# TritonDataCenter/containerpilot

Measured on AMD Instinct MI355X. Metric: events/sec, higher is better.
Workload: dtype n/a (CPU daemon, no tensor math; see BASELINE.json north_star); 1 GPU; model=containerpilot daemon, BASELINE stress shape scaled to 550 jobs, jobs=550, watches=50, parallelism=1 independent daemons (1/rank)

## Files before the change

### cpp/include/cpilot/jobs.hpp

```cpp
#pragma once

#include <functional>
#include <memory>
#include <string>
#include <vector>

#include "cpilot/command.hpp"
#include "cpilot/discovery.hpp"
#include "cpilot/events.hpp"
#include "cpilot/json.hpp"
#include "cpilot/probe.hpp"
#include "cpilot/timing.hpp"

namespace cpilot {

constexpr int kUnlimited = -1;

enum class JobStatus {
  Idle = 0,
  Unknown,
  Healthy,
  Unhealthy,
  Maintenance,
  AlwaysHealthy,
  Completed,
};
const char* jobStatusString(JobStatus s);

struct JobConfig {
  std::string name;
  CommandPtr exec;

  int port = 0;
  std::string initialStatus;
  std::vector<std::string> tags;
  std::shared_ptr<ServiceDefinition> serviceDefinition;

  CommandPtr healthCheckExec;
  health::ProbePtr healthProbe;
// ... 101 lines not shown
```

### cpp/include/cpilot/loop.hpp

```cpp
#pragma once

#include <sys/types.h>

#include <chrono>
#include <cstdint>
#include <deque>
#include <functional>
#include <map>
#include <memory>
#include <mutex>
#include <queue>
#include <vector>

namespace cpilot {

using Clock = std::chrono::steady_clock;
using TimePoint = Clock::time_point;
using Ns = std::chrono::nanoseconds;

std::function<void()> timedItem(const char* tag, std::function<void()> fn);
void dumpItemTags();

void resetThreadScheduling();

class Loop {
 public:
  using FdCallback = std::function<void(uint32_t epollEvents)>;
  using TimerCallback = std::function<void()>;
  using ChildCallback = std::function<void(int waitStatus)>;

  Loop();
  ~Loop();

  Loop(const Loop&) = delete;
  Loop& operator=(const Loop&) = delete;

  void watchFd(int fd, uint32_t events, FdCallback cb);
  void modifyFd(int fd, uint32_t events);
  void unwatchFd(int fd);

  uint64_t addTimeout(Ns delay, TimerCallback cb);
  uint64_t addInterval(Ns interval, TimerCallback cb, Ns initialDelay = Ns(-1));
  void cancelTimer(uint64_t id);

  void defer(std::function<void()> fn);

  void post(std::function<void()> fn);

  void watchChild(pid_t pid, ChildCallback cb);
  void reapChildren();
  void notifyChildExit(pid_t pid, int status);

  static void postIfLive(Loop* loop, uint64_t id, std::function<void()> fn);
  uint64_t id() const { return id_; }

  void run();
  void stop();

  bool stopped() const { return stopped_; }

 private:
  struct Timer {
    uint64_t id;
    TimePoint deadline;
    Ns interval;
    TimerCallback cb;
    bool canceled = false;
  };
  struct TimerCmp {
    bool operator()(const std::shared_ptr<Timer>& a,
                    const std::shared_ptr<Timer>& b) const {
      return a->deadline > b->deadline;
    }
  };

  void armTimerFd();
  void fireDueTimers();
  void drainDeferred();
  void drainPosted();

  uint64_t id_ = 0;
  int epfd_ = -1;
  int timerfd_ = -1;
  int wakeupFds_[2] = {-1, -1};
  bool stopped_ = false;

  std::map<int, FdCallback> fdCallbacks_;
  std::priority_queue<std::shared_ptr<Timer>,
                      std::vector<std::shared_ptr<Timer>>, TimerCmp>
      timers_;
  std::map<uint64_t, std::shared_ptr<Timer>> timersById_;
  uint64_t nextTimerId_ = 1;

  std::deque<std::function<void()>> deferred_;

  std::mutex postedMu_;
  std::deque<std::function<void()>> posted_;

  std::map<pid_t, ChildCallback> children_;
  std::map<pid_t, int> unclaimedExits_;
};

}
```

### cpp/include/cpilot/spawner.hpp

```cpp
#pragma once

#include <sys/types.h>

#include <cstdint>
#include <deque>
#include <functional>
#include <map>
#include <memory>
#include <mutex>
#include <string>
#include <thread>
#include <vector>

#include "cpilot/loop.hpp"

namespace cpilot {

class Spawner {
 public:
  using SpawnCb = std::function<void(pid_t pid, int err)>;

  static Spawner& global();

  void spawn(Loop& loop, const std::string& execPath,
             const std::vector<std::string>& args,
             std::shared_ptr<const std::vector<std::string>> baseEnv,
// ... 4 lines not shown

  size_t backlog();
  bool overloaded();

 private:
  Spawner();
  struct Helper {
    int sock = -1;
    pid_t pid = -1;
    bool dead = false;
    std::deque<std::pair<std::vector<char>, int>> overflow;
    std::mutex sendMu;
  };
  struct Pending {
    Loop* loop;
    uint64_t loopId;
    SpawnCb cb;
    size_t helperIdx;
  };

  bool launchHelper(Helper* h);
  void flushOverflow(size_t idx);
  void readerMain();
  void handleMessage(size_t idx, const char* buf, size_t len);
  void helperDied(size_t idx);
  bool sendRequest(Helper& h, const std::vector<char>& buf, int fd);
  void wakeReader();

  std::string helperPath_;
  std::vector<std::unique_ptr<Helper>> helpers_;
  size_t nextHelper_ = 0;

  std::mutex mu_;
  std::map<uint32_t, Pending> pending_;
  uint32_t nextReqId_ = 1;
  std::map<pid_t, std::pair<Loop*, uint64_t>> pidLoops_;

  int wakeFds_[2] = {-1, -1};
  std::thread reader_;
};

}
```

### cpp/src/discovery.cpp

```cpp
#include "cpilot/discovery.hpp"

#include <algorithm>
#include <cstdlib>
#include <thread>

#include "cpilot/decode.hpp"
#include "cpilot/http.hpp"
#include "cpilot/log.hpp"

namespace cpilot {

namespace {

void parseRawURI(const std::string& raw, std::string* address,
                 std::string* scheme) {
  *scheme = "http";
  *address = raw;
  if (raw.rfind("http://", 0) == 0) {
    *address = raw.substr(7);
  } else if (raw.rfind("https://", 0) == 0) {
    *address = raw.substr(8);
    *scheme = "https";
  }
}
// ... 134 lines not shown
    blockingReg_ = std::make_shared<BlockingReg>();
  for (int i = 0; i < 4; i++)
    workers_.emplace_back([this] { workerMain(); });
}

void ConsulBackend::stop() {
  {
    std::lock_guard<std::mutex> l(mu_);
    if (stopping_ && workers_.empty()) return;
    stopping_ = true;
  }
  {
    std::lock_guard<std::mutex> l(blockingReg_->mu);
    blockingReg_->stopping = true;
    for (auto& t : blockingReg_->tokens) t->cancel();
  }
  cv_.notify_all();
  for (auto& t : workers_) t.join();
  workers_.clear();
}

void ConsulBackend::workerMain() {
  resetThreadScheduling();
  while (true) {
    std::function<void()> task;
    {
      std::unique_lock<std::mutex> l(mu_);
      cv_.wait(l, [this] { return stopping_ || !tasks_.empty(); });
      if (stopping_ && tasks_.empty()) return;
      auto& front = tasks_.front();
      if (!front.first.empty()) queuedKeys_.erase(front.first);
      task = std::move(front.second);
      tasks_.pop_front();
    }
    task();
  }
}

bool ConsulBackend::enqueue(const std::string& key,
                            std::function<void()> task) {
  {
    std::lock_guard<std::mutex> l(mu_);
    if (stopping_) return false;
    if (!key.empty() && !queuedKeys_.insert(key).second) return false;
    if (tasks_.size() >= 10000) {
      if (++dropped_ % 1000 == 1)
// ... 173 lines not shown
                                          HealthBlockingCb cb) {
  std::string path = "/v1/health/service/" + urlEncode(name) + "?passing=1";
  if (!tag.empty()) path += "&tag=" + urlEncode(tag);
  if (!dc.empty()) path += "&dc=" + urlEncode(dc);
  path += "&index=" + std::to_string(lastIndex) +
          "&wait=" + std::to_string(waitSeconds) + "s";
  auto token = std::make_shared<http::CancelToken>();
  auto reg = blockingReg_;
  {
    std::lock_guard<std::mutex> l(reg->mu);
    if (reg->stopping) {
      loop_->post([cb] { cb(false, {}, 0); });
      return;
    }
    reg->tokens.insert(token);
  }
  std::string target = address_;
  std::string tokenHdr = token_;
  http::TlsOptions tls = tls_;
  Loop* loop = loop_;
  std::thread([reg, target, tokenHdr, tls, path, cb, loop, token,
               waitSeconds] {
    resetThreadScheduling();
    std::map<std::string, std::string> headers;
    if (!tokenHdr.empty()) headers["X-Consul-Token"] = tokenHdr;
    auto res = http::request(target, "GET", path, "", "application/json",
                             headers, (waitSeconds + 10) * 1000, &tls,
                             token.get());
    {
      std::lock_guard<std::mutex> l(reg->mu);
      reg->tokens.erase(token);
    }
    bool ok = res.ok && res.status == 200 && !token->cancelled();
    uint64_t index = 0;
    auto it = res.headers.find("x-consul-index");
    if (it != res.headers.end())
      index = strtoull(it->second.c_str(), nullptr, 10);
    std::vector<ServiceEntry> entries;
    if (ok) entries = parseHealthEntries(res.body, &ok);
    loop->post([cb, ok, index, entries = std::move(entries)]() mutable {
      cb(ok, std::move(entries), index);
    });
  }).detach();
}

bool ConsulBackend::compareAndSwap(const std::string& service,
// ... 68 lines not shown
```

### cpp/src/events.cpp

```cpp
#include "cpilot/events.hpp"

#include <algorithm>
#include <cstdio>

#include "cpilot/log.hpp"

namespace cpilot {

const Event GlobalStartup{EventCode::Startup, "global"};
const Event GlobalShutdown{EventCode::Shutdown, "global"};
const Event NonEvent{EventCode::None, ""};
const Event GlobalEnterMaintenance{EventCode::EnterMaintenance, "global"};
const Event GlobalExitMaintenance{EventCode::ExitMaintenance, "global"};
const Event QuitByTest{EventCode::Quit, "closed"};

const char* eventCodeString(EventCode code) {
  switch (code) {
    case EventCode::None: return "None";
    case EventCode::ExitSuccess: return "ExitSuccess";
    case EventCode::ExitFailed: return "ExitFailed";
    case EventCode::Stopping: return "Stopping";
    case EventCode::Stopped: return "Stopped";
    case EventCode::StatusHealthy: return "StatusHealthy";
    case EventCode::StatusUnhealthy: return "StatusUnhealthy";
// ... 66 lines not shown
        tombstones_ = true;
      }
    }
  };
  tombstone(wildcard_);
  for (auto& kv : bySource_) tombstone(kv.second);
  for (auto& kv : byCode_) tombstone(kv.second);
}

void Bus::publish(Event event) {
  LOG_DEBUG("event: %s", event.str().c_str());
  if (event.code != EventCode::Metric) {
    eventsCounter_->inc({eventCodeString(event.code), event.source});
  }
  published_++;
  ring_[(head_ + 1) % (int)ring_.size()] = event;
  int old = head_;
  head_ = (head_ + 1) % (int)ring_.size();
  if (old != -1 && head_ == tail_) tail_ = (tail_ + 1) % (int)ring_.size();

  queue_.emplace_back(std::move(event), Clock::now());
  if (!drainScheduled_) {
    drainScheduled_ = true;
    loop_.defer([self = shared_from_this()] { self->drain(); });
  }
}

void Bus::drain() {
  drainScheduled_ = false;
  constexpr auto kBudget = std::chrono::milliseconds(2);
  TimePoint start = Clock::now();
  size_t n = queue_.size();
  for (size_t i = 0; i < n && !queue_.empty(); i++) {
    if ((i & 63) == 63 && Clock::now() - start >= kBudget) break;
    auto [event, publishedAt] = std::move(queue_.front());
    queue_.pop_front();
    double latency =
        std::chrono::duration<double>(Clock::now() - publishedAt).count();
    dispatchHist_->observe(latency);
    static const bool latDebug = cpilotDebugEnv("CPILOT_LOOP_DEBUG");
    if (latDebug && latency > 0.004)
      fprintf(stderr, "slow dispatch: %s waited %.1f ms (queue %zu)\n",
              event.str().c_str(), latency * 1e3, queue_.size());
    latencySeen_++;
    if (latencyWindow_.size() < latencyCap_) {
      latencyWindow_.push_back(latency);
    } else {
      uint64_t slot = latencyRng_() % latencySeen_;
      if (slot < latencyCap_) latencyWindow_[slot] = latency;
    }
    size_t srcHash = std::hash<std::string>{}(event.source);
    uint64_t seq = ++seq_;
    uint64_t batch = 0;
    deliverList(wildcard_, event, srcHash, seq, &batch);
    auto codeIt = byCode_.find((int)event.code);
    if (codeIt != byCode_.end())
      deliverList(codeIt->second, event, srcHash, seq, &batch);
    auto srcIt = bySource_.find(srcHash);
    if (srcIt != bySource_.end())
      deliverList(srcIt->second, event, srcHash, seq, &batch);
    if (batch) deliveriesCounter_->inc({}, (double)batch);
  }
  if (tombstones_) compactIndexes();
  if (!queue_.empty() && !drainScheduled_) {
    drainScheduled_ = true;
    loop_.defer([self = shared_from_this()] { self->drain(); });
  }
}

void Bus::deliverList(std::vector<Subscriber*>& list, const Event& event,
                      size_t srcHash, uint64_t seq, uint64_t* batch) {
  size_t bound = list.size();
  for (size_t si = 0; si < bound; si++) {
    Subscriber* s = list[si];
    if (!s || s->busSeq_ == seq) continue;
    s->busSeq_ = seq;
    delivered_++;
    (*batch)++;
    s->onEventHashed(event, srcHash);
  }
}

void Bus::compactIndexes() {
  auto compact = [](std::vector<Subscriber*>& list) {
    list.erase(std::remove(list.begin(), list.end(), nullptr), list.end());
  };
  compact(wildcard_);
  for (auto it = bySource_.begin(); it != bySource_.end();) {
    compact(it->second);
    it = it->second.empty() ? bySource_.erase(it) : std::next(it);
// ... 27 lines not shown
```

### cpp/src/jobs.cpp

```cpp
#include "cpilot/jobs.hpp"

#include <unistd.h>

#include <cstring>

#include "cpilot/decode.hpp"
#include "cpilot/ips.hpp"
#include "cpilot/log.hpp"
#include "cpilot/spawner.hpp"

namespace cpilot {

const char* jobStatusString(JobStatus s) {
  switch (s) {
    case JobStatus::Healthy: return "healthy";
    case JobStatus::Unhealthy: return "unhealthy";
    case JobStatus::Maintenance: return "maintenance";
    case JobStatus::AlwaysHealthy: return "healthy";
    case JobStatus::Completed: return "completed";
    default: return "unknown";
  }
}


// ... 505 lines not shown
      startTimeout_(cfg->whenTimeout),
      startsRemain_(cfg->whenStartsLimit),
      stoppingWaitEvent_(cfg->stoppingWaitEvent),
      stoppingTimeout_(cfg->stoppingTimeout),
      heartbeat_(cfg->heartbeatInterval),
      restartLimit_(cfg->restartLimit),
      restartsRemain_(cfg->restartLimit),
      frequency_(cfg->freqInterval) {
  heartbeatSource_ = name_ + ".heartbeat";
  runEverySource_ = name_ + ".run-every";
  healthCheckName_ =
      healthCheckExec_ ? healthCheckExec_->name() : ("check." + name_);
  stoppingTimeoutSource_ = name_ + ".stopping-timeout";
  std::hash<std::string> h;
  hName_ = h(name_);
  hHeartbeat_ = h(heartbeatSource_);
  hRunEvery_ = h(runEverySource_);
  hCheck_ = h(healthCheckName_);
  if (name_ == "containerpilot") {
    status_ = JobStatus::AlwaysHealthy;
  }
}

Subscription Job::subscription() const {
  Subscription sub;
  sub.all = false;
  sub.sources = {name_,          healthCheckName_,
                 heartbeatSource_, runEverySource_,
                 stoppingTimeoutSource_, name_ + ".wait-timeout"};
  if (!startEvent_.source.empty()) sub.sources.push_back(startEvent_.source);
  if (stoppingWaitEvent_ != NonEvent)
    sub.sources.push_back(stoppingWaitEvent_.source);
  sub.codes = {EventCode::Quit, EventCode::Shutdown,
               EventCode::EnterMaintenance, EventCode::ExitMaintenance,
               EventCode::Signal};
  return sub;
}

void Job::run(Loop& loop, std::shared_ptr<Bus> bus,
              std::function<void()> completedCb) {
  loop_ = &loop;
  bus_ = std::move(bus);
  completedCb_ = std::move(completedCb);
  auto self = shared_from_this();

  auto phase = [this](Duration interval) {
    uint64_t h = std::hash<std::string>{}(name_);
    return Duration(interval.count() / 2 +
                    (Ns::rep)(h % 1000) * interval.count() / 2000);
  };

  if (frequency_ > Duration(0)) {
    freqTimer_ = loop.addInterval(frequency_, [this, self] {
      LOG_DEBUG("timer: {TimerExpired %s.run-every}", name_.c_str());
      processEvent(Event{EventCode::TimerExpired, runEverySource_});
    }, phase(frequency_));
  }
  if (heartbeat_ > Duration(0)) {
    heartbeatTimer_ = loop.addInterval(heartbeat_, [this, self] {
      if (name_ != "containerpilot")
        LOG_DEBUG("timer: {TimerExpired %s.heartbeat}", name_.c_str());
      processEvent(Event{EventCode::TimerExpired, heartbeatSource_});
    }, phase(heartbeat_));
  }
  if (service_ && !service_->initialStatus.empty()) {
    regRetryTimer_ = loop.addInterval(std::chrono::seconds(1), [this, self] {
      if (service_->wasRegistered) {
        loop_->cancelTimer(regRetryTimer_);
        regRetryTimer_ = 0;
        return;
      }
      checkRegistration();
// ... 276 lines not shown
```

### cpp/src/loop.cpp

```cpp
#include "cpilot/loop.hpp"

#include <fcntl.h>
#include <sched.h>
#include <sys/resource.h>
#include <sys/epoll.h>
#include <sys/timerfd.h>
#include <sys/wait.h>
#include <unistd.h>

#include <cstdio>
#include <cstring>
#include <algorithm>
#include <set>
#include <stdexcept>

#include "cpilot/log.hpp"

namespace cpilot {

void resetThreadScheduling() {
  struct sched_param sp;
  memset(&sp, 0, sizeof(sp));
  sched_setscheduler(0, SCHED_OTHER, &sp);
  setpriority(PRIO_PROCESS, 0, 0);
}

namespace {
std::mutex& liveLoopsMu() {
// ... 30 lines not shown
    fn();
    auto& slot = itemTags()[t];
    slot.ms +=
        std::chrono::duration<double, std::milli>(Clock::now() - t0).count();
    slot.count++;
  };
}

void dumpItemTags() {
  for (auto& kv : itemTags())
    fprintf(stderr, "  item tag %s: %.0fms over %llu (avg %.1fus)\n",
            kv.first.c_str(), kv.second.ms,
            (unsigned long long)kv.second.count,
            kv.second.count ? kv.second.ms * 1000 / kv.second.count : 0.0);
  itemTags().clear();
}

void Loop::postIfLive(Loop* loop, uint64_t id, std::function<void()> fn) {
  std::lock_guard<std::mutex> l(liveLoopsMu());
  auto it = liveLoops().find(loop);
  if (it != liveLoops().end() && it->second == id) loop->post(std::move(fn));
}

Loop::Loop() {
  {
    std::lock_guard<std::mutex> l(liveLoopsMu());
    id_ = nextLoopId();
    liveLoops()[this] = id_;
  }
  epfd_ = epoll_create1(EPOLL_CLOEXEC);
  if (epfd_ < 0) throw std::runtime_error("epoll_create1 failed");
  timerfd_ = timerfd_create(CLOCK_MONOTONIC, TFD_NONBLOCK | TFD_CLOEXEC);
  if (timerfd_ < 0) throw std::runtime_error("timerfd_create failed");
  if (pipe2(wakeupFds_, O_NONBLOCK | O_CLOEXEC) != 0)
    throw std::runtime_error("pipe2 failed");

  watchFd(timerfd_, EPOLLIN, [this](uint32_t) {
    uint64_t expirations;
    while (read(timerfd_, &expirations, sizeof(expirations)) > 0) {
    }
    fireDueTimers();
  });
  watchFd(wakeupFds_[0], EPOLLIN, [this](uint32_t) {
    char buf[256];
    while (read(wakeupFds_[0], buf, sizeof(buf)) > 0) {
    }
    drainPosted();
  });
}

Loop::~Loop() {
  {
    std::lock_guard<std::mutex> l(liveLoopsMu());
    liveLoops().erase(this);
  }
  if (epfd_ >= 0) close(epfd_);
  if (timerfd_ >= 0) close(timerfd_);
  if (wakeupFds_[0] >= 0) close(wakeupFds_[0]);
  if (wakeupFds_[1] >= 0) close(wakeupFds_[1]);
}

void Loop::watchFd(int fd, uint32_t events, FdCallback cb) {
  struct epoll_event ev;
  memset(&ev, 0, sizeof(ev));
  ev.events = events;
  ev.data.fd = fd;
  if (epoll_ctl(epfd_, EPOLL_CTL_ADD, fd, &ev) != 0)
    throw std::runtime_error(std::string("epoll_ctl ADD failed: ") +
                             strerror(errno));
  fdCallbacks_[fd] = std::move(cb);
}

void Loop::modifyFd(int fd, uint32_t events) {
  struct epoll_event ev;
  memset(&ev, 0, sizeof(ev));
  ev.events = events;
  ev.data.fd = fd;
  epoll_ctl(epfd_, EPOLL_CTL_MOD, fd, &ev);
}

void Loop::unwatchFd(int fd) {
  epoll_ctl(epfd_, EPOLL_CTL_DEL, fd, nullptr);
  fdCallbacks_.erase(fd);
}

uint64_t Loop::addTimeout(Ns delay, TimerCallback cb) {
  auto t = std::make_shared<Timer>();
  t->id = nextTimerId_++;
  t->deadline = Clock::now() + delay;
  t->interval = Ns(0);
  t->cb = std::move(cb);
  timersById_[t->id] = t;
  timers_.push(t);
  armTimerFd();
  return t->id;
}

uint64_t Loop::addInterval(Ns interval, TimerCallback cb, Ns initialDelay) {
  if (interval <= Ns(0)) interval = Ns(1);
  if (initialDelay < Ns(0)) initialDelay = interval;
  auto t = std::make_shared<Timer>();
  t->id = nextTimerId_++;
  t->deadline = Clock::now() + initialDelay;
  t->interval = interval;
  t->cb = std::move(cb);
  timersById_[t->id] = t;
  timers_.push(t);
  armTimerFd();
  return t->id;
}

void Loop::cancelTimer(uint64_t id) {
  auto it = timersById_.find(id);
  if (it == timersById_.end()) return;
  it->second->canceled = true;
  timersById_.erase(it);
}

void Loop::defer(std::function<void()> fn) { deferred_.push_back(std::move(fn)); }

void Loop::post(std::function<void()> fn) {
  {
    std::lock_guard<std::mutex> l(postedMu_);
    posted_.push_back(std::move(fn));
  }
  char b = 1;
  ssize_t unused = write(wakeupFds_[1], &b, 1);
  (void)unused;
}

void Loop::watchChild(pid_t pid, ChildCallback cb) {
  auto it = unclaimedExits_.find(pid);
  if (it != unclaimedExits_.end()) {
    int status = it->second;
    unclaimedExits_.erase(it);
    cb(status);
    return;
  }
  children_[pid] = std::move(cb);
}

void Loop::reapChildren() {
  constexpr int kReapBatch = 64;
  int n = 0;
  while (n < kReapBatch) {
    int status = 0;
    pid_t pid = waitpid(-1, &status, WNOHANG);
    if (pid <= 0) return;
    n++;
    notifyChildExit(pid, status);
  }
  defer([this] { reapChildren(); });
}

void Loop::notifyChildExit(pid_t pid, int status) {
  auto it = children_.find(pid);
  if (it != children_.end()) {
    ChildCallback cb = std::move(it->second);
    children_.erase(it);
    cb(status);
  } else {
    unclaimedExits_[pid] = status;
  }
}

void Loop::armTimerFd() {
  while (!timers_.empty() && timers_.top()->canceled) timers_.pop();
  struct itimerspec its;
  memset(&its, 0, sizeof(its));
  if (!timers_.empty()) {
    auto now = Clock::now();
    Ns delta = std::chrono::duration_cast<Ns>(timers_.top()->deadline - now);
    if (delta < Ns(1)) delta = Ns(1);
    its.it_value.tv_sec = delta.count() / 1000000000LL;
    its.it_value.tv_nsec = delta.count() % 1000000000LL;
  }
  timerfd_settime(timerfd_, 0, &its, nullptr);
}

void Loop::fireDueTimers() {
  static const bool stallDebug = cpilotDebugEnv("CPILOT_LOOP_DEBUG");
  auto timeCb = [](Timer* t, const TimerCallback& cb) {
    if (!stallDebug) { cb(); return; }
    TimePoint t0 = Clock::now();
    cb();
    auto ms = std::chrono::duration<double, std::milli>(Clock::now() - t0)
                  .count();
    if (ms > 10.0)
      fprintf(stderr, "timer stall: id=%llu interval_ms=%lld took %.1f ms\n",
              (unsigned long long)t->id,
              (long long)(t->interval.count() / 1000000), ms);
  };
  auto now = Clock::now();
  while (!timers_.empty()) {
    auto t = timers_.top();
    if (t->canceled) {
      timers_.pop();
      continue;
    }
    if (t->deadline > now) break;
    timers_.pop();
    if (t->interval > Ns(0)) {
      t->deadline += t->interval;
      if (t->deadline <= now) {
        auto behind = std::chrono::duration_cast<Ns>(now - t->deadline);
        auto periods = behind.count() / t->interval.count() + 1;
        t->deadline += Ns(periods * t->interval.count());
      }
      timers_.push(t);
      timeCb(t.get(), t->cb);
    } else {
      auto keep = t;
      timersById_.erase(t->id);
      timeCb(keep.get(), keep->cb);
    }
  }
  armTimerFd();
}

void Loop::drainDeferred() {
  size_t n = deferred_.size();
  for (size_t i = 0; i < n && !deferred_.empty(); i++) {
    auto fn = std::move(deferred_.front());
    deferred_.pop_front();
    fn();
  }
}

void Loop::drainPosted() {
  constexpr auto kBudget = std::chrono::milliseconds(2);
  constexpr size_t kHardCap = 4096;
  TimePoint start = Clock::now();
  size_t processed = 0;
  bool more = true;
  while (more && processed < kHardCap &&
         Clock::now() - start < kBudget) {
    std::deque<std::function<void()>> batch;
    {
      std::lock_guard<std::mutex> l(postedMu_);
      for (size_t i = 0; i < 64 && !posted_.empty(); i++) {
        batch.push_back(std::move(posted_.front()));
        posted_.pop_front();
      }
      more = !posted_.empty();
    }
    static const bool itemDebug = cpilotDebugEnv("CPILOT_LOOP_DEBUG");
    if (itemDebug) {
      static double accMs = 0;
      static uint64_t nItems = 0, nSlow = 0;
      static TimePoint lastDump = Clock::now();
      for (auto& fn : batch) {
        TimePoint ti = Clock::now();
        fn();
        double ms = std::chrono::duration<double, std::milli>(
                        Clock::now() - ti).count();
        accMs += ms;
        nItems++;
        if (ms > 0.2) nSlow++;
      }
      if (Clock::now() - lastDump > std::chrono::seconds(5)) {
        fprintf(stderr,
                "posted items: %llu in 5s, total=%.0fms avg=%.1fus "
                "slow(>200us)=%llu\n",
                (unsigned long long)nItems, accMs,
                nItems ? accMs * 1000.0 / nItems : 0.0,
                (unsigned long long)nSlow);
        accMs = 0;
        nItems = nSlow = 0;
        lastDump = Clock::now();
      }
    } else {
      for (auto& fn : batch) fn();
    }
    processed += batch.size();
    if (batch.empty()) break;
  }
  if (more) {
    char b = 1;
    ssize_t unused = write(wakeupFds_[1], &b, 1);
    (void)unused;
  }
}

void Loop::run() {
  stopped_ = false;
  const bool stallDebug = cpilotDebugEnv("CPILOT_LOOP_DEBUG");
  auto probe = [stallDebug](const char* phase, TimePoint t0, int fd = -1) {
    if (!stallDebug) return;
    auto ms = std::chrono::duration<double, std::milli>(Clock::now() - t0)
                  .count();
    if (ms > 10.0)
      fprintf(stderr, "loop stall: %s fd=%d took %.1f ms\n", phase, fd, ms);
  };
  std::vector<struct epoll_event> events(64);
  double accDeferred = 0, accEpoll = 0, accFds = 0, accTimers = 0;
  std::map<int, std::pair<double, uint64_t>> accPerFd;
  uint64_t iters = 0;
  TimePoint lastReport = Clock::now();
  auto acc = [](double* slot, TimePoint t0) {
    *slot += std::chrono::duration<double, std::milli>(Clock::now() - t0)
                 .count();
  };
  while (!stopped_) {
    TimePoint t0 = Clock::now();
    drainDeferred();
    probe("drainDeferred", t0);
    if (stallDebug) acc(&accDeferred, t0);
    if (stopped_) break;
    armTimerFd();
    int timeoutMs = deferred_.empty() ? 1000 : 0;
    TimePoint te = Clock::now();
    int n = epoll_wait(epfd_, events.data(), (int)events.size(), timeoutMs);
    if (stallDebug) acc(&accEpoll, te);
    if (n < 0) {
      if (errno == EINTR) continue;
      LOG_ERROR("epoll_wait: %s", strerror(errno));
      break;
    }
    TimePoint tf = Clock::now();
    for (int i = 0; i < n && !stopped_; i++) {
      int fd = events[i].data.fd;
      auto it = fdCallbacks_.find(fd);
      if (it != fdCallbacks_.end()) {
        FdCallback cb = it->second;
        TimePoint tc = Clock::now();
        cb(events[i].events);
        probe("fdCallback", tc, fd);
        if (stallDebug) {
          auto& slot = accPerFd[fd];
          slot.first += std::chrono::duration<double, std::milli>(
                            Clock::now() - tc).count();
          slot.second++;
        }
      }
    }
    if (stallDebug) acc(&accFds, tf);
    TimePoint tt = Clock::now();
    fireDueTimers();
    probe("fireDueTimers", tt);
    if (stallDebug) {
      acc(&accTimers, tt);
      iters++;
      if (Clock::now() - lastReport > std::chrono::seconds(5)) {
        double secs = std::chrono::duration<double>(Clock::now() -
                                                    lastReport).count();
        fprintf(stderr,
                "loop phases: %.0f it/s deferred=%.0fms epoll=%.0fms "
                "fds=%.0fms timers=%.0fms (per %.1fs)\n",
                iters / secs, accDeferred, accEpoll, accFds, accTimers,
                secs);
        std::vector<std::pair<double, std::pair<int, uint64_t>>> top;
        for (auto& kv : accPerFd)
          top.push_back({kv.second.first, {kv.first, kv.second.second}});
        std::sort(top.rbegin(), top.rend());
        for (size_t k = 0; k < top.size() && k < 4; k++)
          fprintf(stderr, "  top fd %d: %.0fms over %llu events\n",
                  top[k].second.first, top[k].first,
                  (unsigned long long)top[k].second.second);
        dumpItemTags();
        accPerFd.clear();
        accDeferred = accEpoll = accFds = accTimers = 0;
        iters = 0;
        lastReport = Clock::now();
      }
    }
  }
}

void Loop::stop() { stopped_ = true; }

}
```

### cpp/src/spawner.cpp

```cpp
#include "cpilot/spawner.hpp"

#include <fcntl.h>
#include <limits.h>
#include <poll.h>
#include <signal.h>
#include <spawn.h>
#include <string.h>
#include <sys/socket.h>
#include <unistd.h>

#include <cstdio>
#include <cstdlib>

#include "cpilot/log.hpp"
#include "cpilot/spawnproto.hpp"

extern char** environ;

namespace cpilot {

using namespace spawnproto;

namespace {

int defaultHelperCount() {
  if (const char* v = getenv("CPILOT_SPAWN_HELPERS")) {
    int n = atoi(v);
    if (n >= 1 && n <= 64) return n;
  }
  long ncpu = sysconf(_SC_NPROCESSORS_ONLN);
// ... 14 lines not shown
    size_t slash = dir.find_last_of('/');
    if (slash != std::string::npos) {
      std::string candidate = dir.substr(0, slash) + "/cpilot-spawn-helper";
      if (access(candidate.c_str(), X_OK) == 0) return candidate;
    }
  }
  return "cpilot-spawn-helper";
}

bool spawnDebug() {
  static bool on = cpilotDebugEnv("CPILOT_SPAWN_DEBUG");
  return on;
}

}

Spawner& Spawner::global() {
  static Spawner* s = new Spawner();
  return *s;
}

Spawner::Spawner() {
  helperPath_ = findHelperBinary();
  if (pipe2(wakeFds_, O_NONBLOCK | O_CLOEXEC) != 0)
    LOG_ERROR("spawner: pipe2 failed: %s", strerror(errno));
  int n = defaultHelperCount();
  for (int i = 0; i < n; i++) helpers_.push_back(std::make_unique<Helper>());
  for (auto& h : helpers_) {
    if (!launchHelper(h.get())) {
      logging::logf(logging::Level::Fatal,
                    "spawner: cannot launch spawn helper '%s': %s",
                    helperPath_.c_str(), strerror(errno));
    }
  }
  reader_ = std::thread([this] { readerMain(); });
  reader_.detach();
}

bool Spawner::launchHelper(Helper* h) {
  int socks[2];
  if (socketpair(AF_UNIX, SOCK_SEQPACKET | SOCK_CLOEXEC, 0, socks) != 0)
    return false;
  int bufsz = 1 << 20;
  setsockopt(socks[0], SOL_SOCKET, SO_SNDBUF, &bufsz, sizeof(bufsz));
  setsockopt(socks[1], SOL_SOCKET, SO_SNDBUF, &bufsz, sizeof(bufsz));
  fcntl(socks[0], F_SETFL, O_NONBLOCK);

  posix_spawn_file_actions_t actions;
// ... 44 lines not shown
    size_t sent = 0;
    {
      std::lock_guard<std::mutex> sl(h.sendMu);
      for (auto& [buf, fd] : batch) {
        if (!sendRequest(h, buf, fd)) break;
        if (fd >= 0) close(fd);
        sent++;
      }
    }
    if (sent < batch.size()) {
      std::lock_guard<std::mutex> l(mu_);
      for (size_t i = batch.size(); i > sent; i--)
        h.overflow.push_front(std::move(batch[i - 1]));
      return;
    }
  }
}

bool Spawner::overloaded() {
  return backlog() > helpers_.size() * 16;
}

void Spawner::wakeReader() {
  char b = 1;
  ssize_t unused = write(wakeFds_[1], &b, 1);
  (void)unused;
}

void Spawner::spawn(Loop& loop, const std::string& execPath,
                    const std::vector<std::string>& args,
                    std::shared_ptr<const std::vector<std::string>> baseEnv,
                    const std::vector<std::string>& extraEnv, int stdioFd,
                    SpawnCb cb) {
  RequestHeader hdr;
  memset(&hdr, 0, sizeof(hdr));
  hdr.type = kSpawnRequest;
  hdr.argc = 1 + (uint32_t)args.size();
  hdr.envc = (uint32_t)((baseEnv ? baseEnv->size() : 0) + extraEnv.size());
  hdr.wantStdio = stdioFd >= 0 ? 1 : 0;

  size_t size = sizeof(hdr) + execPath.size() + 1;
  for (auto& a : args) size += a.size() + 1;
  if (baseEnv)
    for (auto& e : *baseEnv) size += e.size() + 1;
  for (auto& e : extraEnv) size += e.size() + 1;
  if (size > kMaxRequestBytes) {
    if (stdioFd >= 0) close(stdioFd);
    loop.post([cb] { cb(-1, E2BIG); });
// ... 73 lines not shown
  if (fd >= 0) {
    memset(cmsgBuf, 0, sizeof(cmsgBuf));
    msg.msg_control = cmsgBuf;
    msg.msg_controllen = sizeof(cmsgBuf);
    struct cmsghdr* c = CMSG_FIRSTHDR(&msg);
    c->cmsg_level = SOL_SOCKET;
    c->cmsg_type = SCM_RIGHTS;
    c->cmsg_len = CMSG_LEN(sizeof(int));
    memcpy(CMSG_DATA(c), &fd, sizeof(int));
  }
  while (true) {
    ssize_t n = sendmsg(h.sock, &msg, MSG_NOSIGNAL);
    if (spawnDebug())
      fprintf(stderr, "[spawner] sendmsg fd=%d n=%zd errno=%d\n", h.sock, n,
              n < 0 ? errno : 0);
    if (n >= 0) return true;
    if (errno == EINTR) continue;
    return false;
  }
}

void Spawner::readerMain() {
  resetThreadScheduling();
  std::vector<char> buf(64);
  while (true) {
    std::vector<struct pollfd> fds;
    {
      std::lock_guard<std::mutex> l(mu_);
      for (auto& h : helpers_) {
        short ev = h->dead ? 0 : POLLIN;
        if (!h->dead && !h->overflow.empty()) ev |= POLLOUT;
        fds.push_back({h->sock, ev, 0});
      }
    }
    fds.push_back({wakeFds_[0], POLLIN, 0});
    int rc = poll(fds.data(), (nfds_t)fds.size(), 1000);
    if (spawnDebug() && rc != 0) {
      fprintf(stderr, "[spawner] poll rc=%d", rc);
      for (size_t i = 0; i < fds.size(); i++)
        fprintf(stderr, " fd%d=%x", fds[i].fd, fds[i].revents);
      fprintf(stderr, "\n");
    }
    if (rc < 0) {
      if (errno == EINTR) continue;
      return;
    }
    if (fds.back().revents & POLLIN) {
      char drain[256];
      while (read(wakeFds_[0], drain, sizeof(drain)) > 0) {
      }
    }
    for (size_t i = 0; i + 1 < fds.size(); i++) {
      if (fds[i].revents & POLLOUT) flushOverflow(i);
      if (fds[i].revents & (POLLIN | POLLHUP | POLLERR)) {
        while (true) {
          ssize_t n = recv(fds[i].fd, buf.data(), buf.size(), MSG_DONTWAIT);
          if (n > 0) {
            if (spawnDebug())
              fprintf(stderr, "[spawner] msg from helper %zu len=%zd\n", i, n);
            handleMessage(i, buf.data(), (size_t)n);
            continue;
          }
          if (n < 0 && (errno == EAGAIN || errno == EINTR)) break;
          if (spawnDebug())
            fprintf(stderr, "[spawner] helper %zu died n=%zd errno=%d\n",
                    i, n, errno);
          helperDied(i);
          break;
        }
      }
    }
  }
}

void Spawner::handleMessage(size_t idx, const char* data, size_t len) {
  uint32_t type = 0;
  if (len >= sizeof(uint32_t)) memcpy(&type, data, sizeof(type));
  if (spawnDebug() && type != kSpawnReply && type != kChildExit)
    fprintf(stderr, "[spawner] DROP unknown msg type=%u len=%zu\n", type, len);
  if (type == kSpawnReply && len >= sizeof(Reply)) {
    Reply r;
    memcpy(&r, data, sizeof(r));
    Pending p;
    {
      std::lock_guard<std::mutex> l(mu_);
      auto it = pending_.find(r.reqId);
      if (it == pending_.end()) {
        if (spawnDebug())
          fprintf(stderr, "[spawner] DROP reply for unknown req %u\n",
                  r.reqId);
        return;
      }
      p = std::move(it->second);
      pending_.erase(it);
    }
    if (spawnDebug())
      fprintf(stderr, "[spawner] reply req %u pid %d\n", r.reqId, r.pid);
    if (r.pid > 0) pidLoops_[r.pid] = {p.loop, p.loopId};
    SpawnCb cb = std::move(p.cb);
    pid_t pid = r.pid;
    int err = r.err;
    Loop::postIfLive(p.loop, p.loopId,
                     timedItem("spawncb", [cb, pid, err] { cb(pid, err); }));
  } else if (type == kChildExit && len >= sizeof(ExitNotice)) {
    ExitNotice note;
    memcpy(&note, data, sizeof(note));
    auto it = pidLoops_.find(note.pid);
    if (it == pidLoops_.end()) {
      if (spawnDebug())
        fprintf(stderr, "[spawner] DROP exit notice for unknown pid %d\n",
                note.pid);
      return;
    }
    if (spawnDebug())
      fprintf(stderr, "[spawner] exit pid %d\n", note.pid);
    auto [loop, loopId] = it->second;
    pidLoops_.erase(it);
    pid_t pid = note.pid;
    int status = note.status;
    Loop::postIfLive(loop, loopId, timedItem("exit", [loop, pid, status] {
                       loop->notifyChildExit(pid, status);
                     }));
  }
}

void Spawner::helperDied(size_t idx) {
  std::vector<Pending> lost;
  {
    std::lock_guard<std::mutex> l(mu_);
    Helper& h = *helpers_[idx];
    if (h.dead) return;
    h.dead = true;
    LOG_ERROR("spawner: helper %d (pid %d) died; respawning",
              (int)idx, (int)h.pid);
    for (auto it = pending_.begin(); it != pending_.end();) {
      if (it->second.helperIdx == idx) {
        lost.push_back(std::move(it->second));
        it = pending_.erase(it);
      } else {
        ++it;
      }
    }
    for (auto& [obuf, ofd] : h.overflow)
      if (ofd >= 0) close(ofd);
    h.overflow.clear();
    close(h.sock);
    if (!launchHelper(&h)) {
      LOG_ERROR("spawner: helper respawn failed: %s", strerror(errno));
      h.dead = true;
    }
  }
  for (auto& p : lost) {
    SpawnCb cb = std::move(p.cb);
    Loop::postIfLive(p.loop, p.loopId, [cb] { cb(-1, ECHILD); });
  }
}

}
```

Before: 11000 events/s.

## Cut reactor syscalls with eventfd wakeups, lazy timerfd arming, microtasks and batched spawner reads

```diff
diff --git a/cpp/include/cpilot/jobs.hpp b/cpp/include/cpilot/jobs.hpp
--- a/cpp/include/cpilot/jobs.hpp
+++ b/cpp/include/cpilot/jobs.hpp
@@ -15,6 +15,8 @@
 namespace cpilot {
 
 constexpr int kUnlimited = -1;
+
+Duration timerPhase(const std::string& name, Duration interval);
 
 enum class JobStatus {
   Idle = 0,
diff --git a/cpp/include/cpilot/loop.hpp b/cpp/include/cpilot/loop.hpp
--- a/cpp/include/cpilot/loop.hpp
+++ b/cpp/include/cpilot/loop.hpp
@@ -2,6 +2,7 @@
 
 #include <sys/types.h>
 
+#include <atomic>
 #include <chrono>
 #include <cstdint>
 #include <deque>
@@ -45,14 +46,23 @@
 
   void defer(std::function<void()> fn);
 
+  void soon(std::function<void()> fn);
+
   void post(std::function<void()> fn);
+  void postBatch(std::vector<std::function<void()>> fns);
 
   void watchChild(pid_t pid, ChildCallback cb);
   void reapChildren();
   void notifyChildExit(pid_t pid, int status);
 
   static void postIfLive(Loop* loop, uint64_t id, std::function<void()> fn);
+  static void postBatchIfLive(Loop* loop, uint64_t id,
+                              std::vector<std::function<void()>> fns);
   uint64_t id() const { return id_; }
+
+  uint64_t wakeWrites() const { return wakeWrites_.load(); }
+  uint64_t timerArms() const { return timerArms_; }
+  uint64_t passes() const { return passes_; }
 
   void run();
   void stop();
@@ -74,15 +84,17 @@
     }
   };
 
-  void armTimerFd();
+  bool armTimerFd();
   void fireDueTimers();
   void drainDeferred();
   void drainPosted();
+  void runMicrotasks();
+  void wake();
 
   uint64_t id_ = 0;
   int epfd_ = -1;
   int timerfd_ = -1;
-  int wakeupFds_[2] = {-1, -1};
+  int wakeFd_ = -1;
   bool stopped_ = false;
 
   std::map<int, FdCallback> fdCallbacks_;
@@ -91,11 +103,20 @@
       timers_;
   std::map<uint64_t, std::shared_ptr<Timer>> timersById_;
   uint64_t nextTimerId_ = 1;
+  bool armed_ = false;
+  TimePoint armedDeadline_{};
+  bool timerDirty_ = true;
+  uint64_t timerArms_ = 0;
+  uint64_t passes_ = 0;
 
   std::deque<std::function<void()>> deferred_;
+  std::deque<std::function<void()>> microtasks_;
+  bool inMicrotasks_ = false;
 
   std::mutex postedMu_;
   std::deque<std::function<void()>> posted_;
+  bool wakePending_ = false;
+  std::atomic<uint64_t> wakeWrites_{0};
 
   std::map<pid_t, ChildCallback> children_;
   std::map<pid_t, int> unclaimedExits_;
diff --git a/cpp/include/cpilot/spawner.hpp b/cpp/include/cpilot/spawner.hpp
--- a/cpp/include/cpilot/spawner.hpp
+++ b/cpp/include/cpilot/spawner.hpp
@@ -2,6 +2,7 @@
 
 #include <sys/types.h>
 
+#include <atomic>
 #include <cstdint>
 #include <deque>
 #include <functional>
@@ -52,7 +53,11 @@
   bool launchHelper(Helper* h);
   void flushOverflow(size_t idx);
   void readerMain();
-  void handleMessage(size_t idx, const char* buf, size_t len);
+  struct Incoming {
+    const char* data;
+    size_t len;
+  };
+  void handleMessages(const std::vector<Incoming>& batch);
   void helperDied(size_t idx);
   bool sendRequest(Helper& h, const std::vector<char>& buf, int fd);
   void wakeReader();
@@ -66,7 +71,8 @@
   uint32_t nextReqId_ = 1;
   std::map<pid_t, std::pair<Loop*, uint64_t>> pidLoops_;
 
-  int wakeFds_[2] = {-1, -1};
+  int wakeFd_ = -1;
+  std::atomic<bool> pollDirty_{true};
   std::thread reader_;
 };
 
diff --git a/cpp/src/discovery.cpp b/cpp/src/discovery.cpp
--- a/cpp/src/discovery.cpp
+++ b/cpp/src/discovery.cpp
@@ -1,4 +1,6 @@
 #include "cpilot/discovery.hpp"
+
+#include <pthread.h>
 
 #include <algorithm>
 #include <cstdlib>
@@ -180,6 +182,7 @@
 
 void ConsulBackend::workerMain() {
   resetThreadScheduling();
+  pthread_setname_np(pthread_self(), "cpilot-consul");
   while (true) {
     std::function<void()> task;
     {
@@ -399,6 +402,7 @@
   std::thread([reg, target, tokenHdr, tls, path, cb, loop, token,
                waitSeconds] {
     resetThreadScheduling();
+    pthread_setname_np(pthread_self(), "cpilot-cwatch");
     std::map<std::string, std::string> headers;
     if (!tokenHdr.empty()) headers["X-Consul-Token"] = tokenHdr;
     auto res = http::request(target, "GET", path, "", "application/json",
diff --git a/cpp/src/events.cpp b/cpp/src/events.cpp
--- a/cpp/src/events.cpp
+++ b/cpp/src/events.cpp
@@ -112,21 +112,19 @@
   queue_.emplace_back(std::move(event), Clock::now());
   if (!drainScheduled_) {
     drainScheduled_ = true;
-    loop_.defer([self = shared_from_this()] { self->drain(); });
+    loop_.soon([self = shared_from_this()] { self->drain(); });
   }
 }
 
 void Bus::drain() {
-  drainScheduled_ = false;
   constexpr auto kBudget = std::chrono::milliseconds(2);
   TimePoint start = Clock::now();
-  size_t n = queue_.size();
-  for (size_t i = 0; i < n && !queue_.empty(); i++) {
-    if ((i & 63) == 63 && Clock::now() - start >= kBudget) break;
+  while (!queue_.empty()) {
+    TimePoint now = Clock::now();
+    if (now - start >= kBudget) break;
     auto [event, publishedAt] = std::move(queue_.front());
     queue_.pop_front();
-    double latency =
-        std::chrono::duration<double>(Clock::now() - publishedAt).count();
+    double latency = std::chrono::duration<double>(now - publishedAt).count();
     dispatchHist_->observe(latency);
     static const bool latDebug = cpilotDebugEnv("CPILOT_LOOP_DEBUG");
     if (latDebug && latency > 0.004)
@@ -152,10 +150,9 @@
     if (batch) deliveriesCounter_->inc({}, (double)batch);
   }
   if (tombstones_) compactIndexes();
-  if (!queue_.empty() && !drainScheduled_) {
-    drainScheduled_ = true;
+  drainScheduled_ = !queue_.empty();
+  if (drainScheduled_)
     loop_.defer([self = shared_from_this()] { self->drain(); });
-  }
 }
 
 void Bus::deliverList(std::vector<Subscriber*>& list, const Event& event,
diff --git a/cpp/src/jobs.cpp b/cpp/src/jobs.cpp
--- a/cpp/src/jobs.cpp
+++ b/cpp/src/jobs.cpp
@@ -551,6 +551,12 @@
   }
 }
 
+Duration timerPhase(const std::string& name, Duration interval) {
+  uint64_t h = std::hash<std::string>{}(name);
+  return Duration(interval.count() / 2 +
+                  (Duration::rep)(h % 1000) * interval.count() / 1000);
+}
+
 Subscription Job::subscription() const {
   Subscription sub;
   sub.all = false;
@@ -574,9 +580,7 @@
   auto self = shared_from_this();
 
   auto phase = [this](Duration interval) {
-    uint64_t h = std::hash<std::string>{}(name_);
-    return Duration(interval.count() / 2 +
-                    (Ns::rep)(h % 1000) * interval.count() / 2000);
+    return timerPhase(name_, interval);
   };
 
   if (frequency_ > Duration(0)) {
diff --git a/cpp/src/loop.cpp b/cpp/src/loop.cpp
--- a/cpp/src/loop.cpp
+++ b/cpp/src/loop.cpp
@@ -1,9 +1,12 @@
 #include "cpilot/loop.hpp"
 
 #include <fcntl.h>
+#include <pthread.h>
 #include <sched.h>
+#include <sys/syscall.h>
 #include <sys/resource.h>
 #include <sys/epoll.h>
+#include <sys/eventfd.h>
 #include <sys/timerfd.h>
 #include <sys/wait.h>
 #include <unistd.h>
@@ -80,6 +83,14 @@
   if (it != liveLoops().end() && it->second == id) loop->post(std::move(fn));
 }
 
+void Loop::postBatchIfLive(Loop* loop, uint64_t id,
+                           std::vector<std::function<void()>> fns) {
+  std::lock_guard<std::mutex> l(liveLoopsMu());
+  auto it = liveLoops().find(loop);
+  if (it != liveLoops().end() && it->second == id)
+    loop->postBatch(std::move(fns));
+}
+
 Loop::Loop() {
   {
     std::lock_guard<std::mutex> l(liveLoopsMu());
@@ -90,19 +101,21 @@
   if (epfd_ < 0) throw std::runtime_error("epoll_create1 failed");
   timerfd_ = timerfd_create(CLOCK_MONOTONIC, TFD_NONBLOCK | TFD_CLOEXEC);
   if (timerfd_ < 0) throw std::runtime_error("timerfd_create failed");
-  if (pipe2(wakeupFds_, O_NONBLOCK | O_CLOEXEC) != 0)
-    throw std::runtime_error("pipe2 failed");
+  wakeFd_ = eventfd(0, EFD_NONBLOCK | EFD_CLOEXEC);
+  if (wakeFd_ < 0) throw std::runtime_error("eventfd failed");
 
   watchFd(timerfd_, EPOLLIN, [this](uint32_t) {
     uint64_t expirations;
-    while (read(timerfd_, &expirations, sizeof(expirations)) > 0) {
-    }
+    ssize_t unused = read(timerfd_, &expirations, sizeof(expirations));
+    (void)unused;
+    armed_ = false;
+    timerDirty_ = true;
     fireDueTimers();
   });
-  watchFd(wakeupFds_[0], EPOLLIN, [this](uint32_t) {
-    char buf[256];
-    while (read(wakeupFds_[0], buf, sizeof(buf)) > 0) {
-    }
+  watchFd(wakeFd_, EPOLLIN, [this](uint32_t) {
+    uint64_t count;
+    ssize_t unused = read(wakeFd_, &count, sizeof(count));
+    (void)unused;
     drainPosted();
   });
 }
@@ -114,8 +127,7 @@
   }
   if (epfd_ >= 0) close(epfd_);
   if (timerfd_ >= 0) close(timerfd_);
-  if (wakeupFds_[0] >= 0) close(wakeupFds_[0]);
-  if (wakeupFds_[1] >= 0) close(wakeupFds_[1]);
+  if (wakeFd_ >= 0) close(wakeFd_);
 }
 
 void Loop::watchFd(int fd, uint32_t events, FdCallback cb) {
@@ -150,7 +162,7 @@
   t->cb = std::move(cb);
   timersById_[t->id] = t;
   timers_.push(t);
-  armTimerFd();
+  if (!armed_ || t->deadline < armedDeadline_) timerDirty_ = true;
   return t->id;
 }
 
@@ -164,7 +176,7 @@
   t->cb = std::move(cb);
   timersById_[t->id] = t;
   timers_.push(t);
-  armTimerFd();
+  if (!armed_ || t->deadline < armedDeadline_) timerDirty_ = true;
   return t->id;
 }
 
@@ -172,19 +184,55 @@
   auto it = timersById_.find(id);
   if (it == timersById_.end()) return;
   it->second->canceled = true;
+  if (armed_ && it->second->deadline <= armedDeadline_) timerDirty_ = true;
   timersById_.erase(it);
 }
 
 void Loop::defer(std::function<void()> fn) { deferred_.push_back(std::move(fn)); }
 
+void Loop::soon(std::function<void()> fn) {
+  microtasks_.push_back(std::move(fn));
+}
+
+void Loop::runMicrotasks() {
+  if (inMicrotasks_) return;
+  inMicrotasks_ = true;
+  while (!microtasks_.empty()) {
+    auto fn = std::move(microtasks_.front());
+    microtasks_.pop_front();
+    fn();
+  }
+  inMicrotasks_ = false;
+}
+
+void Loop::wake() {
+  wakeWrites_.fetch_add(1, std::memory_order_relaxed);
+  uint64_t one = 1;
+  ssize_t unused = write(wakeFd_, &one, sizeof(one));
+  (void)unused;
+}
+
 void Loop::post(std::function<void()> fn) {
+  bool first;
   {
     std::lock_guard<std::mutex> l(postedMu_);
     posted_.push_back(std::move(fn));
-  }
-  char b = 1;
-  ssize_t unused = write(wakeupFds_[1], &b, 1);
-  (void)unused;
+    first = !wakePending_;
+    wakePending_ = true;
+  }
+  if (first) wake();
+}
+
+void Loop::postBatch(std::vector<std::function<void()>> fns) {
+  if (fns.empty()) return;
+  bool first;
+  {
+    std::lock_guard<std::mutex> l(postedMu_);
+    for (auto& fn : fns) posted_.push_back(std::move(fn));
+    first = !wakePending_;
+    wakePending_ = true;
+  }
+  if (first) wake();
 }
 
 void Loop::watchChild(pid_t pid, ChildCallback cb) {
@@ -207,6 +255,7 @@
     if (pid <= 0) return;
     n++;
     notifyChildExit(pid, status);
+    runMicrotasks();
   }
   defer([this] { reapChildren(); });
 }
@@ -222,18 +271,29 @@
   }
 }
 
-void Loop::armTimerFd() {
+bool Loop::armTimerFd() {
+  if (!timerDirty_) return false;
   while (!timers_.empty() && timers_.top()->canceled) timers_.pop();
   struct itimerspec its;
   memset(&its, 0, sizeof(its));
-  if (!timers_.empty()) {
-    auto now = Clock::now();
-    Ns delta = std::chrono::duration_cast<Ns>(timers_.top()->deadline - now);
-    if (delta < Ns(1)) delta = Ns(1);
+  if (timers_.empty()) {
+    timerDirty_ = false;
+    if (!armed_) return false;
+    armed_ = false;
+  } else {
+    TimePoint deadline = timers_.top()->deadline;
+    Ns delta = std::chrono::duration_cast<Ns>(deadline - Clock::now());
+    if (delta < Ns(1)) return true;
+    timerDirty_ = false;
+    if (armed_ && armedDeadline_ == deadline) return false;
+    armed_ = true;
+    armedDeadline_ = deadline;
     its.it_value.tv_sec = delta.count() / 1000000000LL;
     its.it_value.tv_nsec = delta.count() % 1000000000LL;
   }
+  timerArms_++;
   timerfd_settime(timerfd_, 0, &its, nullptr);
+  return false;
 }
 
 void Loop::fireDueTimers() {
@@ -272,8 +332,9 @@
       timersById_.erase(t->id);
       timeCb(keep.get(), keep->cb);
     }
-  }
-  armTimerFd();
+    timerDirty_ = true;
+    runMicrotasks();
+  }
 }
 
 void Loop::drainDeferred() {
@@ -282,6 +343,7 @@
     auto fn = std::move(deferred_.front());
     deferred_.pop_front();
     fn();
+    runMicrotasks();
   }
 }
 
@@ -301,6 +363,7 @@
         posted_.pop_front();
       }
       more = !posted_.empty();
+      if (!more) wakePending_ = false;
     }
     static const bool itemDebug = cpilotDebugEnv("CPILOT_LOOP_DEBUG");
     if (itemDebug) {
@@ -310,6 +373,7 @@
       for (auto& fn : batch) {
         TimePoint ti = Clock::now();
         fn();
+        runMicrotasks();
         double ms = std::chrono::duration<double, std::milli>(
                         Clock::now() - ti).count();
         accMs += ms;
@@ -328,20 +392,21 @@
         lastDump = Clock::now();
       }
     } else {
-      for (auto& fn : batch) fn();
+      for (auto& fn : batch) {
+        fn();
+        runMicrotasks();
+      }
     }
     processed += batch.size();
     if (batch.empty()) break;
   }
-  if (more) {
-    char b = 1;
-    ssize_t unused = write(wakeupFds_[1], &b, 1);
-    (void)unused;
-  }
+  if (more) wake();
 }
 
 void Loop::run() {
   stopped_ = false;
+  if (syscall(SYS_gettid) != getpid())
+    pthread_setname_np(pthread_self(), "cpilot-reactor");
   const bool stallDebug = cpilotDebugEnv("CPILOT_LOOP_DEBUG");
   auto probe = [stallDebug](const char* phase, TimePoint t0, int fd = -1) {
     if (!stallDebug) return;
@@ -354,6 +419,7 @@
   double accDeferred = 0, accEpoll = 0, accFds = 0, accTimers = 0;
   std::map<int, std::pair<double, uint64_t>> accPerFd;
   uint64_t iters = 0;
+  uint64_t lastWakes = wakeWrites(), lastArms = timerArms_;
   TimePoint lastReport = Clock::now();
   auto acc = [](double* slot, TimePoint t0) {
     *slot += std::chrono::duration<double, std::milli>(Clock::now() - t0)
@@ -365,8 +431,10 @@
     probe("drainDeferred", t0);
     if (stallDebug) acc(&accDeferred, t0);
     if (stopped_) break;
-    armTimerFd();
-    int timeoutMs = deferred_.empty() ? 1000 : 0;
+    runMicrotasks();
+    if (stopped_) break;
+    bool timerDue = armTimerFd();
+    int timeoutMs = (deferred_.empty() && !timerDue) ? 1000 : 0;
     TimePoint te = Clock::now();
     int n = epoll_wait(epfd_, events.data(), (int)events.size(), timeoutMs);
     if (stallDebug) acc(&accEpoll, te);
@@ -383,6 +451,7 @@
         FdCallback cb = it->second;
         TimePoint tc = Clock::now();
         cb(events[i].events);
+        runMicrotasks();
         probe("fdCallback", tc, fd);
         if (stallDebug) {
           auto& slot = accPerFd[fd];
@@ -396,6 +465,7 @@
     TimePoint tt = Clock::now();
     fireDueTimers();
     probe("fireDueTimers", tt);
+    passes_++;
     if (stallDebug) {
       acc(&accTimers, tt);
       iters++;
@@ -407,6 +477,12 @@
                 "fds=%.0fms timers=%.0fms (per %.1fs)\n",
                 iters / secs, accDeferred, accEpoll, accFds, accTimers,
                 secs);
+        uint64_t wakes = wakeWrites();
+        fprintf(stderr, "  loop counters: wake writes=%llu timerfd arms=%llu\n",
+                (unsigned long long)(wakes - lastWakes),
+                (unsigned long long)(timerArms_ - lastArms));
+        lastWakes = wakes;
+        lastArms = timerArms_;
         std::vector<std::pair<double, std::pair<int, uint64_t>>> top;
         for (auto& kv : accPerFd)
           top.push_back({kv.second.first, {kv.first, kv.second.second}});
diff --git a/cpp/src/spawner.cpp b/cpp/src/spawner.cpp
--- a/cpp/src/spawner.cpp
+++ b/cpp/src/spawner.cpp
@@ -3,9 +3,11 @@
 #include <fcntl.h>
 #include <limits.h>
 #include <poll.h>
+#include <pthread.h>
 #include <signal.h>
 #include <spawn.h>
 #include <string.h>
+#include <sys/eventfd.h>
 #include <sys/socket.h>
 #include <unistd.h>
 
@@ -66,8 +68,8 @@
 
 Spawner::Spawner() {
   helperPath_ = findHelperBinary();
-  if (pipe2(wakeFds_, O_NONBLOCK | O_CLOEXEC) != 0)
-    LOG_ERROR("spawner: pipe2 failed: %s", strerror(errno));
+  wakeFd_ = eventfd(0, EFD_NONBLOCK | EFD_CLOEXEC);
+  if (wakeFd_ < 0) LOG_ERROR("spawner: eventfd failed: %s", strerror(errno));
   int n = defaultHelperCount();
   for (int i = 0; i < n; i++) helpers_.push_back(std::make_unique<Helper>());
   for (auto& h : helpers_) {
@@ -158,8 +160,9 @@
 }
 
 void Spawner::wakeReader() {
-  char b = 1;
-  ssize_t unused = write(wakeFds_[1], &b, 1);
+  pollDirty_ = true;
+  uint64_t one = 1;
+  ssize_t unused = write(wakeFd_, &one, sizeof(one));
   (void)unused;
 }
 
@@ -279,18 +282,26 @@
 
 void Spawner::readerMain() {
   resetThreadScheduling();
-  std::vector<char> buf(64);
+  pthread_setname_np(pthread_self(), "cpilot-spawnrd");
+  constexpr unsigned kBatch = 32;
+  constexpr size_t kMsgBytes = 64;
+  std::vector<char> bufs(kBatch * kMsgBytes);
+  struct iovec iovs[kBatch];
+  struct mmsghdr msgs[kBatch];
+  std::vector<Incoming> batch;
+  batch.reserve(kBatch);
+  std::vector<struct pollfd> fds;
   while (true) {
-    std::vector<struct pollfd> fds;
-    {
+    if (pollDirty_.exchange(false)) {
+      fds.clear();
       std::lock_guard<std::mutex> l(mu_);
       for (auto& h : helpers_) {
         short ev = h->dead ? 0 : POLLIN;
         if (!h->dead && !h->overflow.empty()) ev |= POLLOUT;
-        fds.push_back({h->sock, ev, 0});
-      }
-    }
-    fds.push_back({wakeFds_[0], POLLIN, 0});
+        fds.push_back({h->dead ? -1 : h->sock, ev, 0});
+      }
+      fds.push_back({wakeFd_, POLLIN, 0});
+    }
     int rc = poll(fds.data(), (nfds_t)fds.size(), 1000);
     if (spawnDebug() && rc != 0) {
       fprintf(stderr, "[spawner] poll rc=%d", rc);
@@ -303,81 +314,120 @@
       return;
     }
     if (fds.back().revents & POLLIN) {
-      char drain[256];
-      while (read(wakeFds_[0], drain, sizeof(drain)) > 0) {
-      }
+      uint64_t count;
+      ssize_t unused = read(wakeFd_, &count, sizeof(count));
+      (void)unused;
     }
     for (size_t i = 0; i + 1 < fds.size(); i++) {
-      if (fds[i].revents & POLLOUT) flushOverflow(i);
+      if (fds[i].revents & POLLOUT) {
+        flushOverflow(i);
+        pollDirty_ = true;
+      }
       if (fds[i].revents & (POLLIN | POLLHUP | POLLERR)) {
         while (true) {
-          ssize_t n = recv(fds[i].fd, buf.data(), buf.size(), MSG_DONTWAIT);
-          if (n > 0) {
+          memset(msgs, 0, sizeof(msgs));
+          for (unsigned k = 0; k < kBatch; k++) {
+            iovs[k] = {bufs.data() + k * kMsgBytes, kMsgBytes};
+            msgs[k].msg_hdr.msg_iov = &iovs[k];
+            msgs[k].msg_hdr.msg_iovlen = 1;
+          }
+          int n = recvmmsg(fds[i].fd, msgs, kBatch, MSG_DONTWAIT, nullptr);
+          if (n < 0 && (errno == EAGAIN || errno == EINTR)) break;
+          bool eof = n <= 0;
+          batch.clear();
+          for (int k = 0; k < n; k++) {
+            if (msgs[k].msg_len == 0) {
+              eof = true;
+              break;
+            }
             if (spawnDebug())
-              fprintf(stderr, "[spawner] msg from helper %zu len=%zd\n", i, n);
-            handleMessage(i, buf.data(), (size_t)n);
-            continue;
+              fprintf(stderr, "[spawner] msg from helper %zu len=%u\n", i,
+                      msgs[k].msg_len);
+            batch.push_back({bufs.data() + k * kMsgBytes, msgs[k].msg_len});
           }
-          if (n < 0 && (errno == EAGAIN || errno == EINTR)) break;
+          handleMessages(batch);
+          if (eof) {
+            if (spawnDebug())
+              fprintf(stderr, "[spawner] helper %zu died n=%d errno=%d\n",
+                      i, n, errno);
+            helperDied(i);
+            break;
+          }
+          if ((unsigned)n < kBatch) break;
+        }
+      }
+    }
+  }
+}
+
+void Spawner::handleMessages(const std::vector<Incoming>& batch) {
+  if (batch.empty()) return;
+  struct Out {
+    Loop* loop;
+    uint64_t loopId;
+    std::function<void()> fn;
+  };
+  std::vector<Out> out;
+  out.reserve(batch.size());
+  {
+    std::lock_guard<std::mutex> l(mu_);
+    for (auto& m : batch) {
+      uint32_t type = 0;
+      if (m.len >= sizeof(uint32_t)) memcpy(&type, m.data, sizeof(type));
+      if (type == kSpawnReply && m.len >= sizeof(Reply)) {
+        Reply r;
+        memcpy(&r, m.data, sizeof(r));
+        auto it = pending_.find(r.reqId);
+        if (it == pending_.end()) {
           if (spawnDebug())
-            fprintf(stderr, "[spawner] helper %zu died n=%zd errno=%d\n",
-                    i, n, errno);
-          helperDied(i);
-          break;
+            fprintf(stderr, "[spawner] DROP reply for unknown req %u\n",
+                    r.reqId);
+          continue;
         }
-      }
-    }
-  }
-}
-
-void Spawner::handleMessage(size_t idx, const char* data, size_t len) {
-  uint32_t type = 0;
-  if (len >= sizeof(uint32_t)) memcpy(&type, data, sizeof(type));
-  if (spawnDebug() && type != kSpawnReply && type != kChildExit)
-    fprintf(stderr, "[spawner] DROP unknown msg type=%u len=%zu\n", type, len);
-  if (type == kSpawnReply && len >= sizeof(Reply)) {
-    Reply r;
-    memcpy(&r, data, sizeof(r));
-    Pending p;
-    {
-      std::lock_guard<std::mutex> l(mu_);
-      auto it = pending_.find(r.reqId);
-      if (it == pending_.end()) {
+        Pending p = std::move(it->second);
+        pending_.erase(it);
         if (spawnDebug())
-          fprintf(stderr, "[spawner] DROP reply for unknown req %u\n",
-                  r.reqId);
-        return;
-      }
-      p = std::move(it->second);
-      pending_.erase(it);
-    }
-    if (spawnDebug())
-      fprintf(stderr, "[spawner] reply req %u pid %d\n", r.reqId, r.pid);
-    if (r.pid > 0) pidLoops_[r.pid] = {p.loop, p.loopId};
-    SpawnCb cb = std::move(p.cb);
-    pid_t pid = r.pid;
-    int err = r.err;
-    Loop::postIfLive(p.loop, p.loopId,
-                     timedItem("spawncb", [cb, pid, err] { cb(pid, err); }));
-  } else if (type == kChildExit && len >= sizeof(ExitNotice)) {
-    ExitNotice note;
-    memcpy(&note, data, sizeof(note));
-    auto it = pidLoops_.find(note.pid);
-    if (it == pidLoops_.end()) {
-      if (spawnDebug())
-        fprintf(stderr, "[spawner] DROP exit notice for unknown pid %d\n",
-                note.pid);
-      return;
-    }
-    if (spawnDebug())
-      fprintf(stderr, "[spawner] exit pid %d\n", note.pid);
-    auto [loop, loopId] = it->second;
-    pidLoops_.erase(it);
-    pid_t pid = note.pid;
-    int status = note.status;
-    Loop::postIfLive(loop, loopId, timedItem("exit", [loop, pid, status] {
-                       loop->notifyChildExit(pid, status);
-                     }));
+          fprintf(stderr, "[spawner] reply req %u pid %d\n", r.reqId, r.pid);
+        if (r.pid > 0) pidLoops_[r.pid] = {p.loop, p.loopId};
+        SpawnCb cb = std::move(p.cb);
+        pid_t pid = r.pid;
+        int err = r.err;
+        out.push_back({p.loop, p.loopId,
+                       timedItem("spawncb", [cb, pid, err] { cb(pid, err); })});
+      } else if (type == kChildExit && m.len >= sizeof(ExitNotice)) {
+        ExitNotice note;
+        memcpy(&note, m.data, sizeof(note));
+        auto it = pidLoops_.find(note.pid);
+        if (it == pidLoops_.end()) {
+          if (spawnDebug())
+            fprintf(stderr, "[spawner] DROP exit notice for unknown pid %d\n",
+                    note.pid);
+          continue;
+        }
+        if (spawnDebug())
+          fprintf(stderr, "[spawner] exit pid %d\n", note.pid);
+        auto [loop, loopId] = it->second;
+        pidLoops_.erase(it);
+        pid_t pid = note.pid;
+        int status = note.status;
+        out.push_back({loop, loopId, timedItem("exit", [loop, pid, status] {
+                         loop->notifyChildExit(pid, status);
+                       })});
+      } else if (spawnDebug()) {
+        fprintf(stderr, "[spawner] DROP unknown msg type=%u len=%zu\n", type,
+                m.len);
+      }
+    }
+  }
+  std::vector<std::function<void()>> fns;
+  for (size_t i = 0; i < out.size();) {
+    size_t j = i;
+    fns.clear();
+    while (j < out.size() && out[j].loop == out[i].loop &&
+           out[j].loopId == out[i].loopId)
+      fns.push_back(std::move(out[j++].fn));
+    Loop::postBatchIfLive(out[i].loop, out[i].loopId, std::move(fns));
+    i = j;
   }
 }
 
@@ -406,6 +456,7 @@
       LOG_ERROR("spawner: helper respawn failed: %s", strerror(errno));
       h.dead = true;
     }
+    pollDirty_ = true;
   }
   for (auto& p : lost) {
     SpawnCb cb = std::move(p.cb);
```

New measurement: 10990 events/s. About the same (-0.1%).
